# pySTEPS/pysteps

Measured on AMD Instinct MI355X. Metric: Mpixels*leadsteps/s (LK+semilag) at 4096x4096 fp32, higher is better.
Workload: dtype f32

## Files before the change

pysteps_amd/csrc/common.h:

```cpp
#pragma once

#include <hip/hip_runtime.h>

#include <cmath>
#include <cstdarg>
#include <cstddef>
#include <cstdint>
#include <cstdio>
#include <mutex>

#include "../../include/pysteps_hip.h"
#include "entry.h"
#include "scratch.h"

#ifdef PSH_DEBUG
#include <cassert>
#define PSH_DASSERT(cond) assert(cond)
#else
#define PSH_DASSERT(cond) ((void)0)
#endif

namespace psh {

constexpr int kNumXcd = 8;
// ... 40 lines not shown
}
template <class F> auto with_real(void *p, bool f64, F &&f) {
  return f64 ? f(static_cast<double *>(p)) : f(static_cast<float *>(p));
}

int check_semilag(int m, int n, int T, int n_iter, int order_and_mode);

struct FieldStats {
  double min_finite = INFINITY, max_finite = -INFINITY;
  double nonfinite = 0, neg_inf = 0, pos_inf = 0, count = 0;
  double nanmin() const {
    if (neg_inf > 0) return -INFINITY;
    if (nonfinite < count) return min_finite;
    return pos_inf > 0 ? INFINITY : NAN;
  }
};
int field_stats_full(const float *in_dev, size_t n, FieldStats *st);
int field_stats_full_f64(const double *in_dev, size_t n, FieldStats *st);
hipError_t launch_convert_f64_f32(const double *in, float *out, size_t n, hipStream_t stream);
hipError_t launch_convert_f32_f64(const float *in, double *out, size_t n, hipStream_t stream);

int pinned_alloc(void **host_ptr, size_t nbytes);
int pinned_free(void *host_ptr);
void pinned_release_cache(bool live = false);

struct SemilagArgs {
  const float *precip;
  const float *vel;
  float *out;
  double *disp;
  const float *scale;
  float first_scale;
  int m, n, T, n_iter, order, resume;
  int row0, rows;
  float outval;
  const float *coef;
  int coef_pad = 0;
  float minval;
  int bmode = 0;
  int spline_order = 3;
  const float *vel_packed = nullptr;
  const float *field_pairs = nullptr;
};
bool semilag_wants_packed(const SemilagArgs &a);
hipError_t launch_pack_velocity(const float *vel, float *uv, size_t plane, hipStream_t stream);
bool semilag_wants_field_pairs(const SemilagArgs &a);
hipError_t launch_pack_field_rows(const float *precip, float *pairs, int m, int n, hipStream_t stream);
hipError_t launch_semilag(const SemilagArgs &a, hipStream_t stream);
bool semilag_window_shape(int m, int n);
int semilag_kernel_choice(int m, int n, int T, int n_iter, int order, bool has_field);
void set_semilag_variant(int v);
void set_members_variant(int v);
void set_lk_fused_nms(int v);
hipError_t spline_prefilter(const float *precip, float *coef, float *tmp, int m, int n, hipStream_t stream, int kind = 0,
                            int npad = 0, int pad_edge = 0, float cval = 0.f, int order = 3);

struct IdwDyn {
  int L;
  int mode;
  float cu, cv;
  float reach;
  int pad[3];
};

bool fft_shape_supported(int m, int n);
int fft_irfft2_weighted(const void *spec_dev, const double *weights_dev, int m, int n, double *out_dev,
                        void *scratch_dev, unsigned long long *min_key_dev = nullptr);

int moments(const double *x_dev, int planes, size_t plane, double2 *stats_dev, hipStream_t stream);

struct IdwArgs {
  const float *xy;
  const float *uv;
  float *out;
  float *out_uv = nullptr;
  int L, k, m, n;
  float x0, dx, y0, dy;
  float inv_res, power, offset, dmax;
  void *scratch = nullptr;
  const IdwDyn *dyn = nullptr;
};
hipError_t launch_idw(const IdwArgs &a, hipStream_t stream);
int idw_resident(const float *xy_dev, const float *values_dev, int capacity, const IdwDyn *dyn_dev, int m, int n,
                 int k, double power, double dist_offset, float *out_dev, float *out_uv_dev = nullptr);
size_t idw_scratch_bytes(int m, int n);
void set_idw_variant(int v);

hipError_t launch_outliers_pooled(const double *xy_dev, const double *uv_dev, const int *count_dev,
                                  int capacity, int k, double thr, unsigned char *flags_dev,
                                  hipStream_t stream);
int lk_track_pool(void *pyramid_handle, const float *points_host, const float *points_dev, const int *npts_dev,
                  int npts, int max_count, double epsilon, double min_eig_threshold, double *pool_xy_dev,
                  double *pool_uv_dev, int *pool_count_dev, int pool_capacity);

int lk_corners_resident(const unsigned char *feature_u8_dev, const float *clean_dev, float *stats_dev, int m, int n,
                        int block_size, int buffer_mask, double quality_level, double min_distance, int max_corners,
                        float *points_dev, int *npoints_dev, int (*before_walk)(void *) = nullptr,
                        void *before_walk_arg = nullptr, int *walk_stats_host = nullptr,
                        unsigned *slots_cleared = nullptr);

size_t lk_prepare_ws_bytes(int m, int n, bool f64);
int lk_prepare_on(hipStream_t stream, void *ws, const void *frame_dev, bool f64, int m, int n, int size_opening,
                  int buffer_mask, float *clean_dev, unsigned char *track_u8_dev, unsigned char *feature_u8_dev,
                  float *stats_dev, unsigned *slots_cleared = nullptr, unsigned long long *keepbits = nullptr);
size_t lk_keepbits_bytes(int m, int n);
size_t lk_slot_bytes();
// ... 23 lines not shown
```

pysteps_amd/csrc/lk.hip:

```cpp
#include <algorithm>
#include <cmath>
#include <cstring>
#include <functional>
#include <vector>

#include "common.h"

#pragma clang fp contract(off)

namespace psh {
namespace {

enum Stat : int {
  kMinAll = 0,
  kNanCount,
  kMaxAll,
  kMinFeat,
  kMaxFeat,
  kEigMax,
  kNumStats = 8
};

constexpr int kRedBlocks = 1024;

// ... 589 lines not shown
  const double fill = dstats[0], hi = dstats[1], flo = dstats[2], fhi = dstats[3];
  const int first_row = buffer_mask > 0 ? (stats[kNanCount] > 0.f ? 2 : 1) : 0;
  const size_t npx = static_cast<size_t>(m) * n;
  const size_t first_feature_px = static_cast<size_t>(first_row) * n;
  const size_t stride = static_cast<size_t>(gridDim.x) * blockDim.x;
  for (size_t p = static_cast<size_t>(blockIdx.x) * blockDim.x + threadIdx.x; p < npx; p += stride) {
    double v = clean[p];
    const bool ok = isfinite(v);
    if (!ok) v = fill;
    trk[p] = quantise_f64(v, fill, hi);
    if (feat) feat[p] = quantise_f64((ok && p >= first_feature_px) ? v : fill, flo, fhi);
  }
}

constexpr int kMaxBlockR = 3;

__device__ __forceinline__ bool px_allowed(const float *__restrict__ clean, int m, int n, int x,
                                           int y, int bm, bool any_nan) {
  if (!any_nan) return true;
  if (bm <= 0) return isfinite(clean[static_cast<size_t>(y) * n + x]);
  const int a = bm / 2;
  for (int j = 0; j < bm; ++j) {
    const int yy = y + j - a;
    if (yy < 0 || yy >= m) continue;
    for (int i = 0; i < bm; ++i) {
      const int xx = x + i - a;
      if (xx < 0 || xx >= n) continue;
      if (!isfinite(clean[static_cast<size_t>(yy) * n + xx])) return false;
    }
  }
  return true;
}

__device__ __forceinline__ float next_lane_f(float v) {
  return __int_as_float(__builtin_amdgcn_update_dpp(0, __float_as_int(v), 0x130 , 0xf, 0xf, true));
}
__device__ __forceinline__ double next_lane_d(double v) {
  const int lo = __builtin_amdgcn_update_dpp(0, __double2loint(v), 0x130, 0xf, 0xf, true);
  const int hi = __builtin_amdgcn_update_dpp(0, __double2hiint(v), 0x130, 0xf, 0xf, true);
  return __hiloint2double(hi, lo);
}
__device__ __forceinline__ bool walk_mirrored(int i, int n) {
  if (i >= 0 && i + 1 < n) return false;
  return reflect101(i + 1, n) != reflect101(reflect101(i, n) + 1, n);
}

constexpr int crn_cols(int block_size) { return 64 - 2 * (block_size / 2 + 1); }

template <int BS, int ROWS>
__global__ __launch_bounds__(256) void lk_corner_response_cols(
    const unsigned char *__restrict__ u8, const float *__restrict__ clean, int m, int n,
    int buffer_mask, const float *__restrict__ stats, float *__restrict__ eig,
    float *__restrict__ partial, Band band, unsigned *__restrict__ slots, int *__restrict__ zero_a, int count_a,
    int *__restrict__ zero_b, int count_b) {
  constexpr int r = BS / 2, H = r + 1, W = crn_cols(BS);
  if (blockIdx.x == 0 && blockIdx.y == 0) {
    for (int i = threadIdx.x; i < count_a; i += 256) zero_a[i] = 0;
    for (int i = threadIdx.x; i < count_b; i += 256) zero_b[i] = 0;
  }
  __shared__ float red[4];
  const int lane = threadIdx.x & 63, wave = __builtin_amdgcn_readfirstlane(threadIdx.x >> 6);
  const int x0 = blockIdx.x * W;
  const int yb = (blockIdx.y * 4 + wave) * ROWS;
  float best = 0.f;
  if (yb < m) {
    const float s = 1.0f / (4.0f * static_cast<float>(BS) * 255.0f), s2 = 2.f * s;
    const int xl = x0 - H + lane;
    const bool neg_x = walk_mirrored(xl + 1, n);
    const float sx = neg_x ? -s : s, sx2 = neg_x ? -s2 : s2;
    const unsigned char *col = u8 + reflect101(xl, n);
    constexpr int kFewRows = 2 * H + 2 > 3 * BS - r ? 2 * H + 2 : 3 * BS - r;
    const bool few_rows = m < kFewRows;
    auto row_of = [&](int y) -> int {
      if (few_rows) return reflect101(y, m);
      y = y < 0 ? -y : y;
      return y >= m ? 2 * m - 2 - y : y;
    };
    auto load_row = [&](int i) -> int { return col[static_cast<size_t>(row_of(yb - H + i)) * n]; };
    auto row_terms = [&](int raw, float &hd, float &g) {
      const float a = static_cast<float>(raw);
      const float c = next_lane_f(a);
      const float b = next_lane_f(c);
      hd = b - a;
      g = (a + b) * s + c * s2;
    };
    const bool any_nan = stats[kNanCount] > 0.f;
    const int x = x0 + lane;
    const bool writer = lane < W && x < n;
    const int rows_out = min(ROWS, m - yb);
    const int last_p = rows_out + BS - 1;
    double ring[3][BS], V[3] = {0.0, 0.0, 0.0};
#pragma unroll
    for (int j = 0; j < BS; ++j) ring[0][j] = ring[1][j] = ring[2][j] = 0.0;
    int raw[BS];
    const int raw0 = load_row(0), raw1 = load_row(1);
#pragma unroll
    for (int j = 0; j < BS; ++j) raw[j] = load_row(2 + j);
    float hd_m, hd_0, g_m, g_0;
    row_terms(raw0, hd_m, g_m);
    row_terms(raw1, hd_0, g_0);
    for (int base = 1; base <= last_p; base += BS) {
      int nxt[BS];
#pragma unroll
      for (int j = 0; j < BS; ++j) nxt[j] = load_row(base + BS + 1 + j);
#pragma unroll
      for (int j = 0; j < BS; ++j) {
        const int p = base + j;
        if (p > last_p) break;
        constexpr int kRingBase = 1;
        const int slot = (kRingBase + j) % BS;
        float hd_p, g_p;
        row_terms(raw[j], hd_p, g_p);
        const float dx = (hd_m + hd_p) * sx + hd_0 * sx2;
        float dy = g_p - g_m;
        const int y_seq = yb - H + p;
        const bool row_mirrored = few_rows ? walk_mirrored(y_seq, m) : (y_seq < 0 || y_seq >= m);
        const unsigned row_sign = row_mirrored ? 0x80000000u : 0u;
        dy = __uint_as_float(__float_as_uint(dy) ^ row_sign);
        const double pxx = static_cast<double>(dx * dx), pxy = static_cast<double>(dx * dy);
        const double pyy = static_cast<double>(dy * dy);
        V[0] += pxx - ring[0][slot];
        V[1] += pxy - ring[1][slot];
        V[2] += pyy - ring[2][slot];
        ring[0][slot] = pxx;
        ring[1][slot] = pxy;
        ring[2][slot] = pyy;
        hd_m = hd_0;
        hd_0 = hd_p;
        g_m = g_0;
        g_0 = g_p;
        if (p >= BS) {
          double w0 = V[0], w1 = V[1], w2 = V[2];
          double t0 = V[0], t1 = V[1], t2 = V[2];
#pragma unroll
          for (int c = 0; c < 2 * r; ++c) {
            t0 = next_lane_d(t0);
            t1 = next_lane_d(t1);
            t2 = next_lane_d(t2);
            w0 += t0;
            w1 += t1;
            w2 += t2;
          }
          const int y = yb + p - BS;
          if (writer) {
            const float a = static_cast<float>(w0) * 0.5f, b = static_cast<float>(w1);
            const float c = static_cast<float>(w2) * 0.5f;
            const float e = (a + c) - sqrtf((a - c) * (a - c) + b * b);
            eig[static_cast<size_t>(y) * n + x] = e;
            if (y >= band.lo && y < band.hi && px_allowed(clean, m, n, x, y, buffer_mask, any_nan))
              best = fmaxf(best, fmaxf(e, 0.f));
          }
        }
      }
#pragma unroll
      for (int j = 0; j < BS; ++j) raw[j] = nxt[j];
    }
  }
  best = wave_max(best);
  if (lane == 0) red[wave] = best;
  __syncthreads();
  if (threadIdx.x == 0) {
    const int b = blockIdx.y * gridDim.x + blockIdx.x;
    const float b_max = fmaxf(fmaxf(red[0], red[1]), fmaxf(red[2], red[3]));
    if (slots) {
      slot_max(slots, kSlEig, b, b_max);
    } else {
      partial[b] = b_max;
    }
  }
}

constexpr int kNmsKeys = 64;

using CornerKeyT = unsigned long long;
__device__ __forceinline__ CornerKeyT nms_key(float val, unsigned addr) {
  return (static_cast<CornerKeyT>(__float_as_uint(val)) << 32) | addr;
}
__device__ __forceinline__ float prev_lane_f(float v) {
  return __int_as_float(__builtin_amdgcn_update_dpp(0, __float_as_int(v), 0x138 , 0xf, 0xf, true));
}

template <int BS, int ROWS>
__global__ __launch_bounds__(256) void lk_corner_response_nms(
    const unsigned char *__restrict__ u8, const float *__restrict__ clean, int m, int n, int buffer_mask,
    const float *__restrict__ stats, float quality, CornerKeyT *__restrict__ out, int cap, Band band,
    unsigned *__restrict__ slots, int *__restrict__ zero_b, int count_b) {
  constexpr int r = BS / 2, H = r + 1, W = crn_cols(BS);
  if (blockIdx.x == 0 && blockIdx.y == 0)
    for (int i = threadIdx.x; i < count_b; i += 256) zero_b[i] = 0;
  __shared__ float red[4];
  const int lane = threadIdx.x & 63, wave = __builtin_amdgcn_readfirstlane(threadIdx.x >> 6);
  int *over_count = reinterpret_cast<int *>(slots + kSlCand * kSlots);
  const int fixed_total = static_cast<int>(gridDim.x * gridDim.y) * 4 * kNmsKeys;
  const int my_slots = (static_cast<int>(blockIdx.y * gridDim.x + blockIdx.x) * 4 + wave) * kNmsKeys;
  const int x0 = blockIdx.x * (W - 2) - 1;
  const int yj = (blockIdx.y * 4 + wave) * ROWS;
  const int yb = yj - 1;
  float best = 0.f;
  float known = fmaxf(slots_max(slots, kSlEig), 0.f);
  int held = 0;
  if (yj < m) {
    const float s = 1.0f / (4.0f * static_cast<float>(BS) * 255.0f), s2 = 2.f * s;
    const int xl = x0 - H + lane;
    const bool neg_x = walk_mirrored(xl + 1, n);
    const float sx = neg_x ? -s : s, sx2 = neg_x ? -s2 : s2;
    const unsigned char *col = u8 + reflect101(xl, n);
    constexpr int kFewRows = 2 * H + 4 > 3 * BS - r + 1 ? 2 * H + 4 : 3 * BS - r + 1;
    const bool few_rows = m < kFewRows;
    auto row_of = [&](int y) -> int {
      if (few_rows) return reflect101(y, m);
      y = y < 0 ? -y : y;
// ... 104 lines not shown
#pragma unroll
      for (int j = 0; j < BS; ++j) raw[j] = nxt[j];
    }
  }
  for (int i = min(held, kNmsKeys) + lane; i < kNmsKeys; i += 64)
    if (my_slots + i < cap) out[my_slots + i] = 0ull;
  best = wave_max(best);
  if (lane == 0) red[wave] = best;
  __syncthreads();
  if (threadIdx.x == 0)
    slot_max(slots, kSlEig, blockIdx.y * gridDim.x + blockIdx.x, fmaxf(fmaxf(red[0], red[1]), fmaxf(red[2], red[3])));
}

__global__ __launch_bounds__(kFinalThreads) void lk_max_final(const float *__restrict__ partial,
                                                              int nb, float *__restrict__ stats,
                                                              int slot, int *__restrict__ zero_a, int count_a,
                                                              int *__restrict__ zero_b, int count_b) {
  __shared__ float smem[16];
  for (int i = threadIdx.x; i < count_a; i += blockDim.x) zero_a[i] = 0;
  for (int i = threadIdx.x; i < count_b; i += blockDim.x) zero_b[i] = 0;
  float a = -INFINITY;
  for (int i = threadIdx.x; i < nb; i += blockDim.x) a = fmaxf(a, partial[i]);
  a = block_reduce<Red::kMax>(a, smem);
  if (threadIdx.x == 0) stats[slot] = a;
}

using CornerKey = unsigned long long;
__host__ __device__ inline CornerKey make_corner_key(float val, unsigned addr) {
#if defined(__HIP_DEVICE_COMPILE__)
  const unsigned bits = __float_as_uint(val);
#else
  unsigned bits;
  std::memcpy(&bits, &val, sizeof(bits));
#endif
  return (static_cast<CornerKey>(bits) << 32) | addr;
}

#ifndef PSH_SEL_WAVES
#define PSH_SEL_WAVES 4
#endif
#ifndef PSH_SEL_GROUPS
#define PSH_SEL_GROUPS 4
#endif
#ifndef PSH_SEL_WIDE
#define PSH_SEL_WIDE 1
#endif
constexpr int kSelWaves = PSH_SEL_WAVES;
constexpr int kSelGroups = PSH_SEL_GROUPS;
constexpr bool kSelWide = PSH_SEL_WIDE != 0;
constexpr int kSelCols = 62;
constexpr int kSelWgRows = kSelWide ? 16 * kSelGroups : 16 * kSelGroups * kSelWaves;
constexpr int kSelWgCols = kSelWide ? kSelCols * kSelWaves : kSelCols;

__global__ __launch_bounds__(64 * kSelWaves) void lk_corner_select(const float *__restrict__ eig,
                                                        const float *__restrict__ clean, int m,
                                                        int n, int buffer_mask, float quality,
                                                        float *__restrict__ stats,
                                                        CornerKey *__restrict__ out, int cap,
                                                        int *__restrict__ count, Band band,
                                                        const unsigned *__restrict__ slots) {
  constexpr int kRows = 16;
  __shared__ unsigned long long s_mask[kSelWaves][kSelGroups * kRows];
  __shared__ int wave_count[kSelWaves];
  __shared__ int block_base;
  const int lane = threadIdx.x & 63, wave = threadIdx.x >> 6;
  const int x = (kSelWide ? (blockIdx.x * kSelWaves + wave) : blockIdx.x) * kSelCols - 1 + lane, xc = x + 1;
  const int y_wave = (kSelWide ? blockIdx.y : (blockIdx.y * kSelWaves + wave)) * (kSelGroups * kRows);
  const float eig_max = slots ? slots_max(slots, kSlEig) : stats[kEigMax];
  if (slots && blockIdx.x == 0 && blockIdx.y == 0 && threadIdx.x == 0) stats[kEigMax] = eig_max;
  const float thr = eig_max * quality;
  const bool any_nan = stats[kNanCount] > 0.f;
  const bool col_in = x >= 0 && x < n;
  const bool col_ok = lane < kSelCols && xc >= 1 && xc < n - 1;
  int mine = 0;
  for (int g = 0; g < kSelGroups; ++g) {
    const int y_first = y_wave + g * kRows;
    if (y_first >= m) {
      if (lane < kRows) s_mask[wave][g * kRows + lane] = 0ull;
      continue;
    }
    float v[kRows + 2], m3[kRows + 2], hmax[kRows + 2];
#pragma unroll
    for (int q = 0; q < kRows + 2; ++q) {
      const int y = y_first - 1 + q;
      v[q] = (col_in && y >= 0 && y < m) ? eig[static_cast<size_t>(y) * n + x] : 0.f;
    }
#pragma unroll
    for (int q = 0; q < kRows + 2; ++q) {
      const float left = v[q], centre = next_lane_f(left), right = next_lane_f(centre);
      hmax[q] = fmaxf(left, right);
      m3[q] = fmaxf(centre, hmax[q]);
      v[q] = centre;
    }
#pragma unroll
    for (int r = 0; r < kRows; ++r) {
      const int yr = y_first + r;
      const float c = v[r + 1];
      bool keep = col_ok && yr >= 1 && yr < m - 1 && yr >= band.lo && yr < band.hi;
      keep = keep && c > thr && c != 0.f;
      keep = keep && !(fmaxf(hmax[r + 1], fmaxf(m3[r], m3[r + 2])) > c);
      keep = keep && px_allowed(clean, m, n, xc, yr, buffer_mask, any_nan);
      const unsigned long long mask = __ballot(keep);
      if (lane == 0) s_mask[wave][g * kRows + r] = mask;
      mine += __popcll(mask);
    }
  }
  if (lane == 0) wave_count[wave] = mine;
  __syncthreads();
  if (threadIdx.x == 0) {
    int total = 0;
    for (int w = 0; w < kSelWaves; ++w) total += wave_count[w];
    block_base = total > 0 ? atomicAdd(count, total) : 0;
  }
  __syncthreads();
  int pos = block_base;
  for (int w = 0; w < wave; ++w) pos += wave_count[w];
  if (mine == 0) return;
  for (int r = 0; r < kSelGroups * kRows; ++r) {
    const unsigned long long mask = s_mask[wave][r];
    if (mask == 0ull) continue;
    const int y = y_wave + r;
    if ((mask >> lane) & 1ull) {
      const int at = pos + __popcll(mask & ((1ull << lane) - 1ull));
      if (at < cap)
        out[at] = make_corner_key(eig[static_cast<size_t>(y) * n + xc], static_cast<unsigned>(y + band.y_org) * n + xc);
    }
    pos += __popcll(mask);
  }
}

constexpr int kPyrRows = 8;

struct PyrPair {
  const unsigned char *src[2];
  unsigned char *dst[2];
};

template <bool FAST>
__device__ __forceinline__ void pyr_rows(const unsigned char *__restrict__ src, unsigned char *__restrict__ dst, int m,
                                         int n, int om, int on, int ox, int oy0, int wx, const int (&off)[11]) {
  auto window = [&](const unsigned char *row) -> uint4 {
    if (FAST) return *reinterpret_cast<const uint4 *>(row + wx);
    unsigned w[4] = {0u, 0u, 0u, 0u};
#pragma unroll
    for (int k = 0; k < 11; ++k) w[(k + 2) >> 2] |= static_cast<unsigned>(row[off[k]]) << (8 * ((k + 2) & 3));
    return make_uint4(w[0], w[1], w[2], w[3]);
  };
  auto hrow = [&](const uint4 d, int h[4]) {
    const unsigned w[4] = {d.x, d.y, d.z, d.w};
    auto b = [&](int k) -> int { return static_cast<int>((w[(k + 2) >> 2] >> (8 * ((k + 2) & 3))) & 0xffu); };
#pragma unroll
    for (int j = 0; j < 4; ++j) h[j] = b(2 * j) + b(2 * j + 4) + 4 * (b(2 * j + 1) + b(2 * j + 3)) + 6 * b(2 * j + 2);
  };
  auto row_ptr = [&](int y) { return src + static_cast<size_t>(reflect101(y, m)) * n; };
  const bool store4 = (on & 3) == 0 && (reinterpret_cast<uintptr_t>(dst) & 3) == 0 && ox + 3 < on;
  constexpr int kHalf = kPyrRows / 2, kIn = 2 * kHalf + 3;
  int h[kIn][4];
#pragma unroll
  for (int half = 0; half < 2; ++half) {
    const int oyh = oy0 + half * kHalf;
    if (oyh >= om) break;
    const int keep = half == 0 ? 0 : 3;
    if (half != 0) {
#pragma unroll
      for (int q = 0; q < 3; ++q)
#pragma unroll
        for (int j = 0; j < 4; ++j) h[q][j] = h[kIn - 3 + q][j];
    }
    uint4 d[kIn];
#pragma unroll
    for (int q = keep; q < kIn; ++q) d[q] = window(row_ptr(2 * oyh - 2 + q));
#pragma unroll
    for (int q = keep; q < kIn; ++q) hrow(d[q], h[q]);
#pragma unroll
    for (int i = 0; i < kHalf; ++i) {
      const int oy = oyh + i;
      if (oy >= om) break;
      unsigned packed = 0;
#pragma unroll
      for (int j = 0; j < 4; ++j) {
// ... 504 lines not shown
    pos += __popcll(mask & ((1ull << lane) - 1ull));
    if (keep && pos < capacity) {
      const float2 p = pts[i], q = next_pts[i];
      pool_xy[pos] = make_double2(p.x, p.y);
      pool_uv[pos] = make_double2(static_cast<double>(q.x - p.x), static_cast<double>(q.y - p.y));
    }
    __syncthreads();
    if (tid == 0) running += wave_total[0] + wave_total[1] + wave_total[2] + wave_total[3];
    __syncthreads();
  }
  if (tid == 0) *pool_count = running;
}

}

dim3 lk_open_grid(int m, int n) { return dim3((n + kOpenColsW - 1) / kOpenColsW, (m + kOpenRowsWG32 - 1) / kOpenRowsWG32); }
void launch_lk_open(dim3 grid, hipStream_t stream, const float *img, int m, int n, int size_opening, int buffer_mask,
                    float *stats, float *clean, float *part, Band band, unsigned *slots = nullptr,
                    unsigned long long *keepbits = nullptr) {
  hipLaunchKernelGGL(lk_open_bits, grid, dim3(256), 0, stream, img, m, n, size_opening, buffer_mask, stats, clean, part,
                     band, slots, keepbits);
}

constexpr int kCrnRows = 32;
dim3 lk_response_grid(int m, int n, int block_size) {
  const int w = crn_cols(block_size), rows = 4 * kCrnRows;
  return dim3((n + w - 1) / w, (m + rows - 1) / rows);
}
dim3 lk_response_nms_grid(int m, int n, int block_size) {
  const int w = crn_cols(block_size) - 2, rows = 4 * kCrnRows;
  return dim3((n + w - 1) / w, (m + rows - 1) / rows);
}
int lk_response_nms_fixed_keys(dim3 grid) { return static_cast<int>(grid.x * grid.y) * 4 * kNmsKeys; }
void launch_lk_response_nms(dim3 grid, hipStream_t stream, int block_size, const unsigned char *u8, const float *clean, int m,
                            int n, int buffer_mask, const float *stats, float quality, CornerKeyT *out, int cap, Band band,
                            unsigned *slots, int *zero_b, int count_b) {
#define PSH_NMS_LAUNCH(BS)                                                                                             \
  hipLaunchKernelGGL((lk_corner_response_nms<BS, kCrnRows>), grid, dim3(256), 0, stream, u8, clean, m, n, buffer_mask, \
                     stats, quality, out, cap, band, slots, zero_b, count_b)
  if (block_size == 1) {
    PSH_NMS_LAUNCH(1);
  } else if (block_size == 3) {
    PSH_NMS_LAUNCH(3);
  } else if (block_size == 5) {
    PSH_NMS_LAUNCH(5);
  } else {
    PSH_NMS_LAUNCH(7);
  }
#undef PSH_NMS_LAUNCH
}
void launch_lk_response(dim3 grid, hipStream_t stream, int block_size, const unsigned char *u8, const float *clean, int m,
                        int n, int buffer_mask, const float *stats, float *eig, float *part, Band band,
                        unsigned *slots = nullptr, int *zero_a = nullptr, int count_a = 0, int *zero_b = nullptr,
                        int count_b = 0) {
#define PSH_CRN_LAUNCH(BS)                                                                                          \
  hipLaunchKernelGGL((lk_corner_response_cols<BS, kCrnRows>), grid, dim3(256), 0, stream, u8, clean, m, n, buffer_mask, \
                     stats, eig, part, band, slots, zero_a, count_a, zero_b, count_b)
  if (block_size == 1) {
    PSH_CRN_LAUNCH(1);
  } else if (block_size == 3) {
    PSH_CRN_LAUNCH(3);
  } else if (block_size == 5) {
    PSH_CRN_LAUNCH(5);
  } else {
    PSH_CRN_LAUNCH(7);
  }
#undef PSH_CRN_LAUNCH
}

static int ensure_lk_ws(size_t nbytes, void **ptr) {
  static void *ws = nullptr;
  const int rc = persistent_device(&ws, nbytes);
  *ptr = ws;
  return rc;
}

size_t lk_prepare_ws_bytes(int m, int n, bool f64) {
  const size_t npx = static_cast<size_t>(m) * n;
  if (f64) {
    const dim3 ogrid((n + kOpenColsW - 1) / kOpenColsW, (m + kOpenRowsWG - 1) / kOpenRowsWG);
    return (npx + 2 * static_cast<size_t>(kRedBlocks) + 3 * static_cast<size_t>(ogrid.x * ogrid.y) + 8) * sizeof(double);
  }
  const dim3 ogrid = lk_open_grid(m, n);
  return kSlotBytes + sizeof(float) * (2 * static_cast<size_t>(kRedBlocks) + 3 * static_cast<size_t>(ogrid.x * ogrid.y));
}
size_t lk_slot_bytes() { return kSlotBytes; }
size_t lk_keepbits_bytes(int m, int n) { return static_cast<size_t>(m) * lk_open_grid(m, n).x * sizeof(unsigned long long); }

int lk_prepare_on(hipStream_t stream, void *ws, const void *frame_dev, bool f64, int m, int n, int size_opening,
                  int buffer_mask, float *clean_dev, unsigned char *track_u8_dev, unsigned char *feature_u8_dev,
                  float *stats_dev, unsigned *slots_cleared, unsigned long long *keepbits) {
  if (m <= 0 || n <= 0) return fail(PSH_EINVAL, "lk_prepare: invalid shape (%d,%d)", m, n);
  if (!frame_dev || !track_u8_dev || !stats_dev || !ws) return fail(PSH_EINVAL, "lk_prepare: NULL pointer");
  if (!clean_dev && (f64 || !keepbits)) return fail(PSH_EINVAL, "lk_prepare: NULL pointer");
  if (size_opening != 0 && size_opening != 3)
    return fail(PSH_EUNSUPPORTED, "lk_prepare: size_opening %d not implemented (0 or 3)", size_opening);
  const size_t npx = static_cast<size_t>(m) * n;
  if (!f64) {
    const float *frame = static_cast<const float *>(frame_dev);
    const dim3 ogrid = lk_open_grid(m, n);
    unsigned *own_slots = static_cast<unsigned *>(ws);
    float *part1 = reinterpret_cast<float *>(static_cast<char *>(ws) + kSlotBytes);
    float *part2 = part1 + 2 * kRedBlocks;
    unsigned *slots = slots_cleared;
    if (!slots) {
      slots = own_slots;
      const hipError_t e = hipMemsetAsync(slots, 0, kSlotBytes, stream);
      if (e != hipSuccess) return fail(PSH_EHIP, "lk_prepare: clearing the statistic slots failed: %s", hipGetErrorString(e));
    }
    hipLaunchKernelGGL(lk_stats1, dim3(kRedBlocks), dim3(256), 0, stream, frame, npx, part1, slots);
    if (clean_dev) {
      launch_lk_open(ogrid, stream, frame, m, n, size_opening, buffer_mask, stats_dev, clean_dev, part2, Band{0, 0, m}, slots);
      const int qgrid = static_cast<int>(std::min<size_t>((npx / 4 + 255) / 256 + 1, 4096));
      hipLaunchKernelGGL(lk_to_u8, dim3(qgrid), dim3(256), 0, stream, clean_dev, m, n, buffer_mask, stats_dev, track_u8_dev,
                         feature_u8_dev, 0, static_cast<const unsigned *>(slots));
    } else {
      launch_lk_open(ogrid, stream, frame, m, n, size_opening, buffer_mask, stats_dev, nullptr, part2, Band{0, 0, m}, slots,
                     keepbits);
      const dim3 qgrid((n + 1023) / 1024, (m + kU8Rows - 1) / kU8Rows);
      const bool vec = n % 4 == 0 && reinterpret_cast<uintptr_t>(frame) % 16 == 0 &&
// ... 97 lines not shown
  hipLaunchKernelGGL(psh::lk_open_final, dim3(1), dim3(psh::kFinalThreads), 0, c.stream, part, nb_open, stats_dev);
  PSH_HIP(hipGetLastError());
  return PSH_OK;
}

int psh_lk_band_to_u8_dev(const float *clean_dev, int m, int n, int e0, int e1, int buffer_mask, const float *stats_dev,
                          unsigned char *track_u8_dev, unsigned char *feature_u8_dev) {
  PSH_ENTER(c);
  if (!clean_dev || !stats_dev || !track_u8_dev) return fail(PSH_EINVAL, "lk_band_to_u8: NULL pointer");
  if (int rc = check_band("lk_band_to_u8", m, n, e0, e1, e0, e1)) return rc;
  const size_t off = static_cast<size_t>(e0) * n, npx = static_cast<size_t>(e1 - e0) * n;
  const int qgrid = static_cast<int>(std::min<size_t>((npx / 4 + 255) / 256 + 1, 4096));
  hipLaunchKernelGGL(psh::lk_to_u8, dim3(qgrid), dim3(256), 0, c.stream, clean_dev + off, e1 - e0, n, buffer_mask,
                     const_cast<float *>(stats_dev), track_u8_dev + off, feature_u8_dev ? feature_u8_dev + off : nullptr, e0,
                     static_cast<const unsigned *>(nullptr));
  PSH_HIP(hipGetLastError());
  return PSH_OK;
}

int psh_lk_band_response_dev(const unsigned char *feature_u8_dev, const float *clean_dev, int m, int n, int e0, int e1,
                             int r0, int r1, int block_size, int buffer_mask, float *stats_dev, float *eig_dev) {
  PSH_ENTER(c);
  if (!feature_u8_dev || !clean_dev || !stats_dev || !eig_dev) return fail(PSH_EINVAL, "lk_band_response: NULL pointer");
  if (int rc = check_band("lk_band_response", m, n, e0, e1, r0, r1)) return rc;
  if (block_size < 1 || block_size > 2 * psh::kMaxBlockR + 1 || (block_size & 1) == 0)
    return fail(PSH_EUNSUPPORTED, "lk_corners: block_size %d not implemented (odd, <= 7)", block_size);
  const int ms = e1 - e0;
  const dim3 rgrid = psh::lk_response_grid(ms, n, block_size);
  const int nb = rgrid.x * rgrid.y;
  void *ws = nullptr;
  if (int rc = psh::ensure_lk_ws(sizeof(float) * static_cast<size_t>(nb), &ws)) return rc;
  float *part = static_cast<float *>(ws);
  const size_t off = static_cast<size_t>(e0) * n;
  const psh::Band band{e0, r0 - e0, r1 - e0};
  psh::launch_lk_response(rgrid, c.stream, block_size, feature_u8_dev + off, clean_dev + off, ms, n, buffer_mask, stats_dev,
                          eig_dev + off, part, band);
  hipLaunchKernelGGL(psh::lk_max_final, dim3(1), dim3(psh::kFinalThreads), 0, c.stream, part, nb, stats_dev,
                     static_cast<int>(psh::kEigMax), static_cast<int *>(nullptr), 0, static_cast<int *>(nullptr), 0);
  PSH_HIP(hipGetLastError());
  return PSH_OK;
}

int psh_lk_band_select_dev(const float *eig_dev, const float *clean_dev, int m, int n, int e0, int e1, int r0, int r1,
                           int buffer_mask, double quality_level, const float *stats_dev,
                           unsigned long long *keys_dev, int cap, int *count_dev) {
  PSH_ENTER(c);
  if (!eig_dev || !clean_dev || !stats_dev || !keys_dev || !count_dev || cap <= 0)
    return fail(PSH_EINVAL, "lk_band_select: invalid argument");
  if (int rc = check_band("lk_band_select", m, n, e0, e1, r0, r1)) return rc;
  const int ms = e1 - e0;
  const size_t off = static_cast<size_t>(e0) * n;
  PSH_HIP(hipMemsetAsync(count_dev, 0, sizeof(int), c.stream));
  PSH_HIP(hipMemsetAsync(keys_dev, 0, static_cast<size_t>(cap) * sizeof(psh::CornerKey), c.stream));
  const dim3 sgrid((n + psh::kSelWgCols - 1) / psh::kSelWgCols, (ms + psh::kSelWgRows - 1) / psh::kSelWgRows);
  hipLaunchKernelGGL(psh::lk_corner_select, sgrid, dim3(64 * psh::kSelWaves), 0, c.stream, eig_dev + off, clean_dev + off, ms, n,
                     buffer_mask, static_cast<float>(quality_level), const_cast<float *>(stats_dev), keys_dev, cap, count_dev,
                     psh::Band{e0, r0 - e0, r1 - e0}, static_cast<const unsigned *>(nullptr));
  PSH_HIP(hipGetLastError());
  return PSH_OK;
}

namespace {
struct CornerJob {
  bool active = false;
  bool host_ordered = false;
  int m = 0, n = 0, cap = 0, max_corners = 0;
  double min_distance = 0.0;
  psh::CornerKey *raw_dev = nullptr;
  hipEvent_t ready = nullptr;
  void *pinned = nullptr;
  void *ws = nullptr;
};
constexpr size_t kPinnedHeader = 64;
constexpr int kMaxCornerJobs = 4;
CornerJob g_corner_jobs[kMaxCornerJobs];
int g_corner_head = 0, g_corner_count = 0;

struct GreedyGrid {
  int cell, gw, gh, n;
  double md2;
  std::vector<int> &head;
  std::vector<int> next, px, py, touched;
  static std::vector<int> &head_store() {
    static thread_local std::vector<int> store;
    return store;
  }
  GreedyGrid(int m, int n_, double min_distance, int max_corners)
      : cell(std::max(1, static_cast<int>(std::lrint(min_distance)))), n(n_),
        md2(min_distance * min_distance), head(head_store()) {
    gw = (n + cell - 1) / cell;
    gh = (m + cell - 1) / cell;
    const size_t cells = static_cast<size_t>(gw) * gh;
    if (head.size() < cells) head.assign(cells, -1);
    next.reserve(max_corners);
    px.reserve(max_corners);
    py.reserve(max_corners);
    touched.reserve(max_corners);
  }
  ~GreedyGrid() {
    for (int cidx : touched) head[cidx] = -1;
  }
  GreedyGrid(const GreedyGrid &) = delete;
  GreedyGrid &operator=(const GreedyGrid &) = delete;
  bool offer(int x, int y) {
    const int xc = x / cell, yc = y / cell;
    for (int yy = std::max(0, yc - 1); yy <= std::min(gh - 1, yc + 1); ++yy)
      for (int xx = std::max(0, xc - 1); xx <= std::min(gw - 1, xc + 1); ++xx)
        for (int q = head[static_cast<size_t>(yy) * gw + xx]; q >= 0; q = next[q]) {
          const double dx = x - px[q], dy = y - py[q];
          if (dx * dx + dy * dy < md2) return false;
        }
    const int id = static_cast<int>(px.size());
    px.push_back(x);
    py.push_back(y);
    const int cidx = yc * gw + xc;
    if (head[cidx] < 0) touched.push_back(cidx);
    next.push_back(head[cidx]);
    head[cidx] = id;
    return true;
  }
};
}

namespace {
static int g_lk_fused_nms = [] {
  const char *e = std::getenv("PYSTEPS_HIP_LK_FUSED_NMS");
  return e ? std::atoi(e) : 0;
}();
}
extern "C++" {
namespace psh {
void set_lk_fused_nms(int v) { g_lk_fused_nms = v; }
}
}
namespace {
struct CornerWs {
  size_t off_part, off_cnt, off_raw, off_ord, bytes;
  int cap, nb;
  dim3 rgrid;
  CornerWs(int m, int n, int block_size) {
    const size_t npx = static_cast<size_t>(m) * n;
    rgrid = psh::lk_response_grid(m, n, block_size);
    nb = rgrid.x * rgrid.y;
    cap = static_cast<int>(std::min<size_t>(npx, 0x7fffffffu));
    cap = static_cast<int>(std::min<size_t>(
        static_cast<size_t>(cap) + psh::lk_response_nms_fixed_keys(psh::lk_response_nms_grid(m, n, block_size)), 0x7fffffffu));
    auto up = [](size_t v) { return (v + 255) & ~static_cast<size_t>(255); };
    off_part = up(npx * sizeof(float));
    off_cnt = up(off_part + static_cast<size_t>(nb) * sizeof(float));
    off_raw = up(off_cnt + sizeof(int));
    off_ord = up(off_raw + static_cast<size_t>(cap) * sizeof(psh::CornerKey));
    bytes = off_ord + psh::corner_order_ws_bytes();
  }
};

int corner_candidates(const CornerWs &w, void *ws, const unsigned char *feature_u8_dev, const float *clean_dev,
                      float *stats_dev, int m, int n, int block_size, int buffer_mask, double quality_level,
                      unsigned *eig_slots = nullptr, const int **count_dev_out = nullptr, int *count_bias_out = nullptr) {
  psh::Context &c = ctx();
  char *base = static_cast<char *>(ws);
  float *eig = reinterpret_cast<float *>(base);
  float *part = reinterpret_cast<float *>(base + w.off_part);
  int *cnt = reinterpret_cast<int *>(base + w.off_cnt);
  psh::CornerKey *raw = reinterpret_cast<psh::CornerKey *>(base + w.off_raw);
  int *ord = reinterpret_cast<int *>(base + w.off_ord);
  const int ord_ints = static_cast<int>(psh::corner_order_clear_bytes() / sizeof(int));
  if (count_dev_out) *count_dev_out = cnt;
  if (eig_slots && count_dev_out && count_bias_out && g_lk_fused_nms) {
    const dim3 ngrid = psh::lk_response_nms_grid(m, n, block_size);
    psh::launch_lk_response_nms(ngrid, c.stream, block_size, feature_u8_dev, clean_dev, m, n, buffer_mask, stats_dev,
                                static_cast<float>(quality_level), raw, w.cap, psh::Band{0, 0, m}, eig_slots, ord, ord_ints);
    *count_dev_out = reinterpret_cast<const int *>(eig_slots + psh::kSlCand * psh::kSlots);
    *count_bias_out = psh::lk_response_nms_fixed_keys(ngrid);
    PSH_HIP(hipGetLastError());
    return PSH_OK;
  }
  if (eig_slots) {
    psh::launch_lk_response(w.rgrid, c.stream, block_size, feature_u8_dev, clean_dev, m, n, buffer_mask, stats_dev, eig,
                            part, psh::Band{0, 0, m}, eig_slots, cnt, 1, ord, ord_ints);
  } else {
    psh::launch_lk_response(w.rgrid, c.stream, block_size, feature_u8_dev, clean_dev, m, n, buffer_mask, stats_dev, eig,
                            part, psh::Band{0, 0, m});
    hipLaunchKernelGGL(psh::lk_max_final, dim3(1), dim3(psh::kFinalThreads), 0, c.stream, part, w.nb, stats_dev,
                       static_cast<int>(psh::kEigMax), cnt, 1, ord, ord_ints);
  }
  const dim3 sgrid((n + psh::kSelWgCols - 1) / psh::kSelWgCols, (m + psh::kSelWgRows - 1) / psh::kSelWgRows);
  hipLaunchKernelGGL(psh::lk_corner_select, sgrid, dim3(64 * psh::kSelWaves), 0, c.stream, eig, clean_dev, m, n, buffer_mask,
                     static_cast<float>(quality_level), stats_dev, raw, w.cap, cnt, psh::Band{0, 0, m},
                     static_cast<const unsigned *>(eig_slots));
  PSH_HIP(hipGetLastError());
  return PSH_OK;
}

int check_corner_args(const unsigned char *feature_u8_dev, const float *clean_dev, const float *stats_dev, int m,
                      int n, int block_size, int max_corners) {
  if (m <= 0 || n <= 0) return fail(PSH_EINVAL, "lk_corners: invalid shape (%d,%d)", m, n);
  if (!feature_u8_dev || !clean_dev || !stats_dev) return fail(PSH_EINVAL, "lk_corners: NULL pointer");
  if (block_size < 1 || block_size > 2 * psh::kMaxBlockR + 1 || (block_size & 1) == 0)
    return fail(PSH_EUNSUPPORTED, "lk_corners: block_size %d not implemented (odd, <= 7)", block_size);
  if (max_corners <= 0) return fail(PSH_EINVAL, "lk_corners: max_corners must be positive");
  if (static_cast<uint64_t>(m) * static_cast<uint64_t>(n) >= (1ull << 31))
    return fail(PSH_EUNSUPPORTED, "lk_corners: more than 2^31 pixels");
  return PSH_OK;
}
}

extern "C++" {
namespace psh {
int lk_corners_resident(const unsigned char *feature_u8_dev, const float *clean_dev, float *stats_dev, int m, int n,
                        int block_size, int buffer_mask, double quality_level, double min_distance, int max_corners,
                        float *points_dev, int *npoints_dev, int (*before_walk)(void *), void *before_walk_arg,
                        int *walk_stats_host, unsigned *slots_cleared) {
  if (int rc = check_corner_args(feature_u8_dev, clean_dev, stats_dev, m, n, block_size, max_corners)) return rc;
  if (!points_dev || !npoints_dev) return fail(PSH_EINVAL, "lk_corners: NULL pointer");
  if (!corner_order_supported(m, n, min_distance, max_corners))
    return fail(PSH_EUNSUPPORTED, "lk_corners: more than %d corners or 65535 rows / columns are ordered on the host",
                corner_order_max_corners());
  Context &c = ctx();
  const CornerWs w(m, n, block_size);
  Scratch ws;
  if (int rc = ws.alloc(w.bytes)) return rc;
  const int *count_dev = nullptr;
  int count_bias = 0;
  int rc = corner_candidates(w, ws.as<void>(), feature_u8_dev, clean_dev, stats_dev, m, n, block_size, buffer_mask, quality_level,
                             slots_cleared, &count_dev, &count_bias);
  if (rc == PSH_OK) {
    char *base = ws.as<char>();
    const hipError_t e = launch_corner_order(
        reinterpret_cast<const CornerKey *>(base + w.off_raw), count_dev, w.cap,
        stats_dev + kEigMax, static_cast<float>(quality_level), n, min_distance, max_corners, base + w.off_ord,
        points_dev, npoints_dev, c.stream, before_walk, before_walk_arg, true,
        count_bias ? slots_cleared + psh::kSlEig * psh::kSlots : nullptr, count_bias, count_bias ? stats_dev + kEigMax : nullptr);
    if (e != hipSuccess) rc = fail(PSH_EHIP, "corner_order launch failed: %s", hipGetErrorString(e));
    if (rc == PSH_OK && walk_stats_host) {
      if (hipMemcpyAsync(walk_stats_host, base + w.off_ord + corner_order_walk_stats_offset(), 13 * sizeof(int),
                         hipMemcpyDeviceToHost, c.stream) != hipSuccess ||
          hipStreamSynchronize(c.stream) != hipSuccess)
        rc = fail(PSH_EHIP, "corner_order statistics copy failed");
    }
  }
  return rc;
}
// ... 471 lines not shown
```

pysteps_amd/csrc/runtime.hip:

```cpp
#include <cmath>
#include <cstdlib>
#include <cstring>
#include <map>
#include <vector>

#include "common.h"
#include "registry.h"

namespace psh {

Context &ctx() {
  static Context c;
  return c;
}

static thread_local char g_err[512] = "";

int fail(int code, const char *fmt, ...) {
  va_list ap;
  va_start(ap, fmt);
  vsnprintf(g_err, sizeof(g_err), fmt, ap);
  va_end(ap);
  return code;
}
// ... 157 lines not shown
[[maybe_unused]] static const int g_side_hook = at_shutdown([] {
  Context &c = ctx();
  if (!c.side) return;
  (void)hipStreamDestroy(c.side);
  (void)hipEventDestroy(c.fork_ev);
  (void)hipEventDestroy(c.join_ev);
  c.side = nullptr;
  c.fork_ev = c.join_ev = nullptr;
});
}
}

int psh_shutdown(void) {
  psh::Context &c = ctx();
  psh::Lock lock(c.mu);
  if (!c.ready) return PSH_OK;
  (void)psh::bind_device(c.device);
  (void)hipStreamSynchronize(c.stream);
  if (c.side) (void)hipStreamSynchronize(c.side);
  psh::registry().release_all();
  (void)hipStreamDestroy(c.stream);
  c.stream = nullptr;
  c.const_next = 0;
  c.mask_generation = 0;
  c.ready = false;
  return PSH_OK;
}

int psh_set_option(const char *key, int value) {
  if (!key) return fail(PSH_EINVAL, "psh_set_option: NULL key");
  if (std::strcmp(key, "semilag_variant") == 0) {
    if (value != 0 && value != 1 && value != 5 && value != 7 && value != 12)
      return fail(PSH_EINVAL,
                  "semilag_variant must be 0 (window kernel where it applies, gather kernels elsewhere), 12 (window kernel "
                  "for every eligible call), 7 (gather kernels: packed {u,v} plane + row-pair field plane), 5 (packed "
                  "velocity only) or 1 (one plane per component, DPP column sharing)");
    psh::set_semilag_variant(value);
    return PSH_OK;
  }
  if (std::strcmp(key, "members_variant") == 0) {
    if (value != 1 && value != 2)
      return fail(PSH_EINVAL, "members_variant must be 2 (two members per thread, default) or 1 (one)");
    psh::set_members_variant(value);
    return PSH_OK;
  }
  if (std::strcmp(key, "idw_variant") == 0) {
    if (value < 0 || value > 1) return fail(PSH_EINVAL, "idw_variant must be 0 (two-level) or 1 (pre-pass per 16x16 tile)");
    psh::set_idw_variant(value);
    return PSH_OK;
  }
  if (std::strcmp(key, "lk_fused_nms") == 0) {
    if (value != 0 && value != 1) return fail(PSH_EINVAL, "lk_fused_nms must be 0 (response + selection passes, default) or 1 (one fused pass)");
    psh::set_lk_fused_nms(value);
    return PSH_OK;
  }
  if (std::strcmp(key, "trim_cache") == 0) {
    psh::Context &c = ctx();
    psh::Lock lock(c.mu);
    if (c.ready) {
      if (int rc = psh::bind_device(c.device)) return rc;
      PSH_HIP(hipStreamSynchronize(c.stream));
      psh::release_cache();
      psh::pinned_release_cache();
    }
    return PSH_OK;
  }
  return fail(PSH_EINVAL, "psh_set_option: unknown option '%s'", key);
}

int psh_field_stats_dev(const float *in_dev, size_t n, double *min_out, double *max_out,
                        double *nonfinite_out, double *nanmin_out);

int psh_device_info(int *device_id, int *cu_count, size_t *hbm_total, size_t *hbm_free,
                    char *name, int name_len) {
  PSH_ENTER(c);
  if (device_id) *device_id = c.device;
  if (cu_count) *cu_count = c.cu_count;
  if (hbm_total || hbm_free) {
    size_t f = 0, t = 0;
    PSH_HIP(hipMemGetInfo(&f, &t));
    if (hbm_total) *hbm_total = t;
    if (hbm_free) *hbm_free = f;
  }
  if (name && name_len > 0) {
    hipDeviceProp_t prop;
    PSH_HIP(hipGetDeviceProperties(&prop, c.device));
    std::snprintf(name, name_len, "%s (%s)", prop.name, prop.gcnArchName);
  }
  return PSH_OK;
}

int psh_malloc(void **dev_ptr, size_t nbytes) {
  PSH_ENTER(c);
  if (!dev_ptr) return fail(PSH_EINVAL, "psh_malloc: NULL out pointer");
  *dev_ptr = nullptr;
  if (nbytes == 0) return PSH_OK;
  nbytes = (nbytes + 255) & ~static_cast<size_t>(255);
  psh::BlockCache &bc = psh::cache();
  auto it = bc.free_blocks.find(nbytes);
  if (it != bc.free_blocks.end() && !it->second.empty()) {
    *dev_ptr = it->second.back();
    it->second.pop_back();
    bc.cached_bytes -= nbytes;
    bc.live[*dev_ptr] = nbytes;
    return PSH_OK;
  }
// ... 260 lines not shown
```

Baseline: 278,800.

## Add row-streaming corner selection kernel with per-tile max skip

Adds a new default corner-selection kernel that streams rows through a register ring, with four columns per lane and ballot-built masks. The response kernel now also records a per-wave tile maximum of the eigenvalue response, and selection skips regions whose tile max is below the quality threshold. This is meant to cut eig reads and NMS work in the selection pass. The old tile kernel is kept as variant 1, and a no-skip variant is variant 2. The change adds a small tile buffer and a global store in the response kernel.

Result: no change. 278,700 (-0.0%).

```diff
diff --git a/pysteps_amd/csrc/common.h b/pysteps_amd/csrc/common.h
--- a/pysteps_amd/csrc/common.h
+++ b/pysteps_amd/csrc/common.h
@@ -116,6 +116,7 @@
 void set_semilag_variant(int v);
 void set_members_variant(int v);
 void set_lk_fused_nms(int v);
+void set_lk_select_variant(int v);
 hipError_t spline_prefilter(const float *precip, float *coef, float *tmp, int m, int n, hipStream_t stream, int kind = 0,
                             int npad = 0, int pad_edge = 0, float cval = 0.f, int order = 3);
 
diff --git a/pysteps_amd/csrc/lk.hip b/pysteps_amd/csrc/lk.hip
--- a/pysteps_amd/csrc/lk.hip
+++ b/pysteps_amd/csrc/lk.hip
@@ -665,7 +665,7 @@
     const unsigned char *__restrict__ u8, const float *__restrict__ clean, int m, int n,
     int buffer_mask, const float *__restrict__ stats, float *__restrict__ eig,
     float *__restrict__ partial, Band band, unsigned *__restrict__ slots, int *__restrict__ zero_a, int count_a,
-    int *__restrict__ zero_b, int count_b) {
+    int *__restrict__ zero_b, int count_b, float *__restrict__ tile_best) {
   constexpr int r = BS / 2, H = r + 1, W = crn_cols(BS);
   if (blockIdx.x == 0 && blockIdx.y == 0) {
     for (int i = threadIdx.x; i < count_a; i += 256) zero_a[i] = 0;
@@ -770,6 +770,7 @@
     }
   }
   best = wave_max(best);
+  if (tile_best != nullptr && yb < m && lane == 0) tile_best[(blockIdx.y * 4 + wave) * gridDim.x + blockIdx.x] = best;
   if (lane == 0) red[wave] = best;
   __syncthreads();
   if (threadIdx.x == 0) {
@@ -980,7 +981,7 @@
 constexpr int kSelWgRows = kSelWide ? 16 * kSelGroups : 16 * kSelGroups * kSelWaves;
 constexpr int kSelWgCols = kSelWide ? kSelCols * kSelWaves : kSelCols;
 
-__global__ __launch_bounds__(64 * kSelWaves) void lk_corner_select(const float *__restrict__ eig,
+__global__ __launch_bounds__(64 * kSelWaves) void lk_corner_select_tiles(const float *__restrict__ eig,
                                                         const float *__restrict__ clean, int m,
                                                         int n, int buffer_mask, float quality,
                                                         float *__restrict__ stats,
@@ -1054,6 +1055,164 @@
         out[at] = make_corner_key(eig[static_cast<size_t>(y) * n + xc], static_cast<unsigned>(y + band.y_org) * n + xc);
     }
     pos += __popcll(mask);
+  }
+}
+
+constexpr int kSelRowCols = 252;
+constexpr int kSelRowRows = 16;
+constexpr int kSelRowDepth = 8;
+constexpr int kSelRowWaves = 4;
+constexpr int kSelRowWgRows = kSelRowRows * kSelRowWaves;
+constexpr int kSelStoreRows = 4;
+static_assert(kSelRowRows % kSelStoreRows == 0, "pass 2 walks whole steps");
+
+template <bool VEC>
+__device__ __forceinline__ int sel_rows_judge(const float *__restrict__ eig, const float *__restrict__ clean, int m, int n,
+                                              int buffer_mask, float thr, bool any_nan, Band band, int x, int y_wave, int lane,
+                                              unsigned long long *masks) {
+  const bool in0 = x < n, in1 = x + 1 < n, in2 = x + 2 < n, in3 = x + 3 < n;
+  const int xc0 = VEC ? min(x, n - 4) : min(x, n - 1), xc1 = min(x + 1, n - 1), xc2 = min(x + 2, n - 1);
+  const int xc3 = min(x + 3, n - 1);
+  auto load_row = [&](int q) -> float4 {
+    const float *row = eig + static_cast<size_t>(min(max(y_wave - 1 + q, 0), m - 1)) * n;
+    if (VEC) return *reinterpret_cast<const float4 *>(row + xc0);
+    return make_float4(row[xc0], row[xc1], row[xc2], row[xc3]);
+  };
+  auto in_image = [&](float4 v, int q) -> float4 {
+    const int y = y_wave - 1 + q;
+    const bool row_in = y >= 0 && y < m;
+    if (VEC) return (row_in && in0) ? v : make_float4(0.f, 0.f, 0.f, 0.f);
+    return make_float4((row_in && in0) ? v.x : 0.f, (row_in && in1) ? v.y : 0.f, (row_in && in2) ? v.z : 0.f,
+                       (row_in && in3) ? v.w : 0.f);
+  };
+  const int rows_here = min(kSelRowRows, m - y_wave);
+  bool col_ok[4];
+#pragma unroll
+  for (int j = 0; j < 4; ++j) col_ok[j] = lane < 63 && x + 1 + j < n - 1;
+  float4 ring[kSelRowDepth];
+#pragma unroll
+  for (int q = 0; q < kSelRowDepth; ++q) ring[q] = load_row(q);
+  float m3_up[4] = {0.f, 0.f, 0.f, 0.f}, c_mid[4] = {0.f, 0.f, 0.f, 0.f}, h_mid[4] = {0.f, 0.f, 0.f, 0.f};
+  float m3_mid[4] = {0.f, 0.f, 0.f, 0.f};
+  int mine = 0;
+#pragma unroll
+  for (int q = 0; q < kSelRowRows + 2; ++q) {
+    const int k = q % kSelRowDepth;
+    const float4 v = in_image(ring[k], q);
+    if (q + kSelRowDepth < kSelRowRows + 2) ring[k] = load_row(q + kSelRowDepth);
+    const float a[6] = {v.x, v.y, v.z, v.w, next_lane_f(v.x), next_lane_f(v.y)};
+    float c_new[4], h_new[4], m3_new[4];
+#pragma unroll
+    for (int j = 0; j < 4; ++j) {
+      c_new[j] = a[j + 1];
+      h_new[j] = fmaxf(a[j], a[j + 2]);
+      m3_new[j] = fmaxf(c_new[j], h_new[j]);
+    }
+    const int r = q - 2, yr = y_wave + r;
+    if (r >= 0 && r < rows_here) {
+      const bool row_ok = yr >= 1 && yr < m - 1 && yr >= band.lo && yr < band.hi;
+#pragma unroll
+      for (int j = 0; j < 4; ++j) {
+        const float c = c_mid[j];
+        bool keep = col_ok[j] && row_ok;
+        keep = keep && c > thr && c != 0.f;
+        keep = keep && !(fmaxf(h_mid[j], fmaxf(m3_up[j], m3_new[j])) > c);
+        const unsigned long long mask = __ballot(keep);
+        if (lane == 0) masks[r * 4 + j] = mask;
+        mine += __popcll(mask);
+      }
+    }
+#pragma unroll
+    for (int j = 0; j < 4; ++j) {
+      m3_up[j] = m3_mid[j];
+      c_mid[j] = c_new[j];
+      h_mid[j] = h_new[j];
+      m3_mid[j] = m3_new[j];
+    }
+  }
+  if (any_nan) {
+    mine = 0;
+    for (int i = 0; i < rows_here * 4; ++i) {
+      unsigned long long mask = masks[i];
+      if (mask == 0ull) continue;
+      const bool keep = ((mask >> lane) & 1ull) != 0ull &&
+                        px_allowed(clean, m, n, x + 1 + (i & 3), y_wave + (i >> 2), buffer_mask, any_nan);
+      mask = __ballot(keep);
+      if (lane == 0) masks[i] = mask;
+      mine += __popcll(mask);
+    }
+  }
+  for (int i = rows_here * 4 + lane; i < kSelRowRows * 4; i += 64) masks[i] = 0ull;
+  return mine;
+}
+
+__global__ __launch_bounds__(64 * kSelRowWaves) void lk_corner_select(
+    const float *__restrict__ eig, const float *__restrict__ clean, int m, int n, int buffer_mask, float quality,
+    float *__restrict__ stats, CornerKey *__restrict__ out, int cap, int *__restrict__ count, Band band,
+    const unsigned *__restrict__ slots, const float *__restrict__ tile_best, int tile_cols, int tile_rows,
+    int tiles_per_row) {
+  __shared__ unsigned long long s_mask[kSelRowWaves][kSelRowRows * 4];
+  __shared__ int wave_count[kSelRowWaves];
+  __shared__ int block_base;
+  const int lane = threadIdx.x & 63, wave = __builtin_amdgcn_readfirstlane(threadIdx.x >> 6);
+  const int x0 = blockIdx.x * kSelRowCols, x = x0 + 4 * lane;
+  const int y_wave = (blockIdx.y * kSelRowWaves + wave) * kSelRowRows;
+  const float eig_max = slots ? slots_max(slots, kSlEig) : stats[kEigMax];
+  if (slots && blockIdx.x == 0 && blockIdx.y == 0 && threadIdx.x == 0) stats[kEigMax] = eig_max;
+  const float thr = eig_max * quality;
+  const bool any_nan = stats[kNanCount] > 0.f;
+  const int xa = x0 + 1, xb = min(x0 + kSelRowCols, n - 2), yb = min(y_wave + kSelRowRows, m) - 1;
+  bool work = y_wave < m && xb >= xa;
+  if (work && tile_best != nullptr) {
+    const int tx0 = xa / tile_cols, ntx = xb / tile_cols - tx0 + 1;
+    const int ty0 = y_wave / tile_rows, total = ntx * (yb / tile_rows - ty0 + 1);
+    bool above = false;
+    for (int i = lane; i < total; i += 64)
+      above = above || tile_best[static_cast<size_t>(ty0 + i / ntx) * tiles_per_row + tx0 + i % ntx] > thr;
+    work = __ballot(above) != 0ull;
+  }
+  int mine = 0;
+  if (!work) {
+    for (int i = lane; i < kSelRowRows * 4; i += 64) s_mask[wave][i] = 0ull;
+  } else {
+    const bool vec = (n & 3) == 0 && (reinterpret_cast<uintptr_t>(eig) & 15) == 0;
+    mine = vec ? sel_rows_judge<true>(eig, clean, m, n, buffer_mask, thr, any_nan, band, x, y_wave, lane, s_mask[wave])
+               : sel_rows_judge<false>(eig, clean, m, n, buffer_mask, thr, any_nan, band, x, y_wave, lane, s_mask[wave]);
+  }
+  if (lane == 0) wave_count[wave] = mine;
+  __syncthreads();
+  if (threadIdx.x == 0) {
+    int total = 0;
+    for (int w = 0; w < kSelRowWaves; ++w) total += wave_count[w];
+    block_base = total > 0 ? atomicAdd(count, total) : 0;
+  }
+  __syncthreads();
+  int pos = block_base;
+  for (int w = 0; w < wave; ++w) pos += wave_count[w];
+  if (mine == 0) return;
+  for (int r0 = 0; r0 < kSelRowRows; r0 += kSelStoreRows) {
+    unsigned long long mk[kSelStoreRows * 4], any = 0ull;
+#pragma unroll
+    for (int i = 0; i < kSelStoreRows * 4; ++i) {
+      mk[i] = s_mask[wave][r0 * 4 + i];
+      any |= mk[i];
+    }
+    if (any == 0ull) continue;
+    float val[kSelStoreRows * 4];
+#pragma unroll
+    for (int i = 0; i < kSelStoreRows * 4; ++i) {
+      const int y = y_wave + r0 + (i >> 2), xc = x + 1 + (i & 3);
+      val[i] = eig[static_cast<size_t>(min(y, m - 1)) * n + min(xc, n - 1)];
+    }
+#pragma unroll
+    for (int i = 0; i < kSelStoreRows * 4; ++i) {
+      const int y = y_wave + r0 + (i >> 2), xc = x + 1 + (i & 3);
+      if ((mk[i] >> lane) & 1ull) {
+        const int at = pos + __popcll(mk[i] & ((1ull << lane) - 1ull));
+        if (at < cap) out[at] = make_corner_key(val[i], static_cast<unsigned>(y + band.y_org) * n + xc);
+      }
+      pos += __popcll(mk[i]);
+    }
   }
 }
 
@@ -1664,10 +1823,10 @@
 void launch_lk_response(dim3 grid, hipStream_t stream, int block_size, const unsigned char *u8, const float *clean, int m,
                         int n, int buffer_mask, const float *stats, float *eig, float *part, Band band,
                         unsigned *slots = nullptr, int *zero_a = nullptr, int count_a = 0, int *zero_b = nullptr,
-                        int count_b = 0) {
+                        int count_b = 0, float *tile_best = nullptr) {
 #define PSH_CRN_LAUNCH(BS)                                                                                          \
   hipLaunchKernelGGL((lk_corner_response_cols<BS, kCrnRows>), grid, dim3(256), 0, stream, u8, clean, m, n, buffer_mask, \
-                     stats, eig, part, band, slots, zero_a, count_a, zero_b, count_b)
+                     stats, eig, part, band, slots, zero_a, count_a, zero_b, count_b, tile_best)
   if (block_size == 1) {
     PSH_CRN_LAUNCH(1);
   } else if (block_size == 3) {
@@ -1678,6 +1837,29 @@
     PSH_CRN_LAUNCH(7);
   }
 #undef PSH_CRN_LAUNCH
+}
+size_t lk_response_tiles(dim3 grid) { return static_cast<size_t>(grid.x) * grid.y * 4; }
+
+static int g_lk_select_variant = [] {
+  const char *e = std::getenv("PYSTEPS_HIP_LK_SELECT_VARIANT");
+  const int v = e ? std::atoi(e) : 0;
+  return v >= 0 && v <= 2 ? v : 0;
+}();
+void set_lk_select_variant(int v) { g_lk_select_variant = v; }
+void launch_lk_select(hipStream_t stream, const float *eig, const float *clean, int m, int n, int buffer_mask, float quality,
+                      float *stats, CornerKey *out, int cap, int *count, Band band, const unsigned *slots,
+                      const float *tile_best = nullptr, int block_size = 1, dim3 rgrid = dim3(1, 1)) {
+  if (g_lk_select_variant == 1) {
+    const dim3 sgrid((n + kSelWgCols - 1) / kSelWgCols, (m + kSelWgRows - 1) / kSelWgRows);
+    hipLaunchKernelGGL(lk_corner_select_tiles, sgrid, dim3(64 * kSelWaves), 0, stream, eig, clean, m, n, buffer_mask,
+                       quality, stats, out, cap, count, band, slots);
+    return;
+  }
+  if (g_lk_select_variant == 2) tile_best = nullptr;
+  const dim3 sgrid(std::max(1, (n - 2 + kSelRowCols - 1) / kSelRowCols), (m + kSelRowWgRows - 1) / kSelRowWgRows);
+  hipLaunchKernelGGL(lk_corner_select, sgrid, dim3(64 * kSelRowWaves), 0, stream, eig, clean, m, n, buffer_mask, quality,
+                     stats, out, cap, count, band, slots, tile_best, crn_cols(block_size), kCrnRows,
+                     static_cast<int>(rgrid.x));
 }
 
 static int ensure_lk_ws(size_t nbytes, void **ptr) {
@@ -1881,10 +2063,9 @@
   const size_t off = static_cast<size_t>(e0) * n;
   PSH_HIP(hipMemsetAsync(count_dev, 0, sizeof(int), c.stream));
   PSH_HIP(hipMemsetAsync(keys_dev, 0, static_cast<size_t>(cap) * sizeof(psh::CornerKey), c.stream));
-  const dim3 sgrid((n + psh::kSelWgCols - 1) / psh::kSelWgCols, (ms + psh::kSelWgRows - 1) / psh::kSelWgRows);
-  hipLaunchKernelGGL(psh::lk_corner_select, sgrid, dim3(64 * psh::kSelWaves), 0, c.stream, eig_dev + off, clean_dev + off, ms, n,
-                     buffer_mask, static_cast<float>(quality_level), const_cast<float *>(stats_dev), keys_dev, cap, count_dev,
-                     psh::Band{e0, r0 - e0, r1 - e0}, static_cast<const unsigned *>(nullptr));
+  psh::launch_lk_select(c.stream, eig_dev + off, clean_dev + off, ms, n, buffer_mask, static_cast<float>(quality_level),
+                        const_cast<float *>(stats_dev), keys_dev, cap, count_dev, psh::Band{e0, r0 - e0, r1 - e0},
+                        static_cast<const unsigned *>(nullptr));
   PSH_HIP(hipGetLastError());
   return PSH_OK;
 }
@@ -1964,7 +2145,7 @@
 }
 namespace {
 struct CornerWs {
-  size_t off_part, off_cnt, off_raw, off_ord, bytes;
+  size_t off_part, off_tile, off_cnt, off_raw, off_ord, bytes;
   int cap, nb;
   dim3 rgrid;
   CornerWs(int m, int n, int block_size) {
@@ -1976,7 +2157,8 @@
         static_cast<size_t>(cap) + psh::lk_response_nms_fixed_keys(psh::lk_response_nms_grid(m, n, block_size)), 0x7fffffffu));
     auto up = [](size_t v) { return (v + 255) & ~static_cast<size_t>(255); };
     off_part = up(npx * sizeof(float));
-    off_cnt = up(off_part + static_cast<size_t>(nb) * sizeof(float));
+    off_tile = up(off_part + static_cast<size_t>(nb) * sizeof(float));
+    off_cnt = up(off_tile + psh::lk_response_tiles(rgrid) * sizeof(float));
     off_raw = up(off_cnt + sizeof(int));
     off_ord = up(off_raw + static_cast<size_t>(cap) * sizeof(psh::CornerKey));
     bytes = off_ord + psh::corner_order_ws_bytes();
@@ -1990,6 +2172,7 @@
   char *base = static_cast<char *>(ws);
   float *eig = reinterpret_cast<float *>(base);
   float *part = reinterpret_cast<float *>(base + w.off_part);
+  float *tiles = reinterpret_cast<float *>(base + w.off_tile);
   int *cnt = reinterpret_cast<int *>(base + w.off_cnt);
   psh::CornerKey *raw = reinterpret_cast<psh::CornerKey *>(base + w.off_raw);
   int *ord = reinterpret_cast<int *>(base + w.off_ord);
@@ -2006,17 +2189,15 @@
   }
   if (eig_slots) {
     psh::launch_lk_response(w.rgrid, c.stream, block_size, feature_u8_dev, clean_dev, m, n, buffer_mask, stats_dev, eig,
-                            part, psh::Band{0, 0, m}, eig_slots, cnt, 1, ord, ord_ints);
+                            part, psh::Band{0, 0, m}, eig_slots, cnt, 1, ord, ord_ints, tiles);
   } else {
     psh::launch_lk_response(w.rgrid, c.stream, block_size, feature_u8_dev, clean_dev, m, n, buffer_mask, stats_dev, eig,
-                            part, psh::Band{0, 0, m});
+                            part, psh::Band{0, 0, m}, nullptr, nullptr, 0, nullptr, 0, tiles);
     hipLaunchKernelGGL(psh::lk_max_final, dim3(1), dim3(psh::kFinalThreads), 0, c.stream, part, w.nb, stats_dev,
                        static_cast<int>(psh::kEigMax), cnt, 1, ord, ord_ints);
   }
-  const dim3 sgrid((n + psh::kSelWgCols - 1) / psh::kSelWgCols, (m + psh::kSelWgRows - 1) / psh::kSelWgRows);
-  hipLaunchKernelGGL(psh::lk_corner_select, sgrid, dim3(64 * psh::kSelWaves), 0, c.stream, eig, clean_dev, m, n, buffer_mask,
-                     static_cast<float>(quality_level), stats_dev, raw, w.cap, cnt, psh::Band{0, 0, m},
-                     static_cast<const unsigned *>(eig_slots));
+  psh::launch_lk_select(c.stream, eig, clean_dev, m, n, buffer_mask, static_cast<float>(quality_level), stats_dev, raw, w.cap,
+                        cnt, psh::Band{0, 0, m}, static_cast<const unsigned *>(eig_slots), tiles, block_size, w.rgrid);
   PSH_HIP(hipGetLastError());
   return PSH_OK;
 }
diff --git a/pysteps_amd/csrc/runtime.hip b/pysteps_amd/csrc/runtime.hip
--- a/pysteps_amd/csrc/runtime.hip
+++ b/pysteps_amd/csrc/runtime.hip
@@ -233,6 +233,14 @@
   if (std::strcmp(key, "lk_fused_nms") == 0) {
     if (value != 0 && value != 1) return fail(PSH_EINVAL, "lk_fused_nms must be 0 (response + selection passes, default) or 1 (one fused pass)");
     psh::set_lk_fused_nms(value);
+    return PSH_OK;
+  }
+  if (std::strcmp(key, "lk_select_variant") == 0) {
+    if (value < 0 || value > 2)
+      return fail(PSH_EINVAL,
+                  "lk_select_variant must be 0 (row-streaming selection pass, tiles under the threshold skipped, default), "
+                  "1 (the tile kernel, 62 columns x 16-row groups per wave) or 2 (row-streaming, no tile skipped)");
+    psh::set_lk_select_variant(value);
     return PSH_OK;
   }
   if (std::strcmp(key, "trim_cache") == 0) {
```
